# PRBonn/RAP

Hardware: AMD Instinct MI355X
Metric: registered points/sec @20 flow steps, 2-view N=4096 (higher is better)
Workload: dtype f32; 1 GPU; configs[1]: batch=32 samples/GPU x 2 views x 4096 pts, 20 Euler flow steps, rap_12 (d=512, H=8), fp32 (exact-fp32 MFMA), rigidity_forcing=on, final per-view SE(3) fit; preset=1, pairs_per_gpu=32, views=2, points_per_view=4096, flow_steps=20, num_layers=12, rigidity_forcing=True

## Files before the change

rap_amd/csrc/api.hip:

```cpp
#include "../../include/rapflow.h"
#include "half.h"
#include "kernels.h"

#include <mutex>
#include <new>
#include <vector>

static thread_local int g_last_hip_error = 0;
void rap_set_last_hip_error(int e) { g_last_hip_error = e; }

#define RAP_PROF_CLASSES 8
struct ProfRec { hipEvent_t a, b; int cls; };
static std::atomic<bool> g_prof_on{false};
static std::mutex g_prof_mu;
static std::vector<ProfRec> g_prof_recs;
static std::vector<hipEvent_t> g_prof_pool;
static size_t g_prof_pool_used = 0;
static const size_t RAP_PROF_MAX_EVENTS = 1u << 19;

static hipEvent_t prof_event() {
  if (g_prof_pool_used < g_prof_pool.size()) return g_prof_pool[g_prof_pool_used++];
  if (g_prof_pool.size() >= RAP_PROF_MAX_EVENTS) return nullptr;
  hipEvent_t e = nullptr;
  if (hipEventCreate(&e) != hipSuccess) return nullptr;
  g_prof_pool.push_back(e);
  g_prof_pool_used++;
  return e;
}
struct ProfScope {
  hipStream_t s; hipEvent_t a = nullptr, b = nullptr; int cls;
  ProfScope(hipStream_t s_, int cls_) : s(s_), cls(cls_) {
    if (!g_prof_on.load(std::memory_order_relaxed)) return;
    std::lock_guard<std::mutex> lock(g_prof_mu);
    a = prof_event(); b = prof_event();
    if (a && b) (void)hipEventRecord(a, s); else a = b = nullptr;
  }
  ~ProfScope() {
    if (a && b) {
      std::lock_guard<std::mutex> lock(g_prof_mu);
      (void)hipEventRecord(b, s); g_prof_recs.push_back({a, b, cls});
    }
  }
};
extern "C" int rap_profile_enable(int on) { g_prof_on.store(on != 0); return RAP_OK; }
extern "C" int rap_profile_reset(void) { std::lock_guard<std::mutex> lock(g_prof_mu); g_prof_recs.clear(); g_prof_pool_used = 0; return RAP_OK; }
extern "C" int rap_profile_collect_ex(float* h_ms_out, int64_t* h_count_out, int32_t n_classes) {
  if (!h_ms_out || !h_count_out || n_classes <= 0) return RAP_ERR_INVALID;
  std::lock_guard<std::mutex> lock(g_prof_mu);
  for (int c = 0; c < n_classes; ++c) { h_ms_out[c] = 0.f; h_count_out[c] = 0; }
  for (const ProfRec& r : g_prof_recs) {
    if (r.cls >= n_classes) continue;
    if (hipEventSynchronize(r.b) != hipSuccess) return RAP_ERR_HIP;
    float ms = 0.f;
    if (hipEventElapsedTime(&ms, r.a, r.b) != hipSuccess) return RAP_ERR_HIP;
    h_ms_out[r.cls] += ms; h_count_out[r.cls] += 1;
  }
  return RAP_OK;
}
extern "C" int rap_profile_collect(float* h_ms_out, int64_t* h_count_out) { return rap_profile_collect_ex(h_ms_out, h_count_out, 3); }

struct LayerW {
  const float* Wqkv[2];
  const float* Wout[2];
  const float* bout[2];
  const float* gq[2];
  const float* gk[2];
  const float* ffn_g;
  const float* ffn_b;
  const float* Wff1p;
  const float* bff1p;
  const float* Wff2;
  const float* bff2;
};

struct LayerWH {
  const u16* Wqkv[2];
  const u16* Wout[2];
  const u16* Wff1p;
  const u16* Wff2;
  float s_qkv[2] = {1.f, 1.f}, s_out[2] = {1.f, 1.f}, s_ff1 = 1.f, s_ff2 = 1.f;
  float g_v[2] = {1.f, 1.f}, g_ff1 = 1.f;
};
struct HalfWeights {
  u16* blob = nullptr;
  std::vector<LayerWH> layers;
};
#define RAP_MAX_LOGIT_BOUND 40.0f

struct rap_model {
  rap_model_desc desc;
  int d, L, H, F, E;
  int Din = 0;
  int Ks = 128;
  int dtype = RAP_DT_F32;
  bool qk_norm = true;
  int resid_dtype = RAP_DT_F32;
  HalfWeights half[4];
  float* logit_bound = nullptr;
  std::vector<uint8_t> bounded;
  int n_bounded = 0;
  float* raw = nullptr;
  float* derived = nullptr;
  const float* anchor_emb;
  const float* emb_bias;
  const float* Wstatic;
  const float* Wx;
  const float *adaW1, *adab1, *adaW2, *adab2, *adaW3, *adab3;
  std::vector<LayerW> layers;
  const float *hW0, *hb0, *hW2, *hb2, *hW4;
  mutable std::mutex cfg_mu;
};

static bool desc_ok(const rap_model_desc* d) {
  if (!d) return false;
  if (d->embed_dim <= 0 || d->embed_dim % 256 != 0 || d->embed_dim > 1024) return false;
  if (d->num_heads * 64 != d->embed_dim) return false;
  if (d->num_layers <= 0 || d->num_layers > 64) return false;
  if (d->local_feat_dim < 0 || d->local_feat_dim % 4 != 0 || d->local_feat_dim > 40) return false;
  return true;
}

extern rap_tuning_t g_rap_gemm_variant;
extern rap_tuning_t g_rap_gemm_stagger;
extern rap_tuning_t g_rap_gemm_splitk;
extern rap_tuning_t g_rap_geglu_fast;
extern rap_tuning_t g_rap_attn_split;
extern rap_tuning_t g_rap_gemm_h16_variant;
extern rap_tuning_t g_rap_attn_h16_variant;
extern rap_tuning_t g_rap_gemm_h16_persistent;
extern rap_tuning_t g_rap_attn_h16_dma;
extern rap_tuning_t g_rap_gemm_f32_persistent;
extern rap_tuning_t g_rap_attn_x2_wpe;
extern rap_tuning_t g_rap_attn_h16_small;
rap_tuning_t g_rap_attn_lpt = 1;
rap_tuning_t g_rap_x2_min_rows = 1024;
rap_tuning_t g_rap_small_fused = 1;
extern rap_tuning_t g_rap_ring_blocks;
rap_tuning_t g_rap_fuse_qknorm = 1;
extern "C" int rap_set_tuning(int32_t key, int32_t value) {
#ifdef RAP_ABLATION_BUILD
  if (key == 0 && (value == 16 || value == 32 || value == 48)) { g_rap_gemm_variant = value; return RAP_OK; }
  if (key == 2 && (value == 0 || value == 1 || value == 14)) { g_rap_gemm_h16_variant = value; return RAP_OK; }
  if (key == 3 && (value == 0 || value == 5)) { g_rap_attn_h16_variant = value; return RAP_OK; }
  if (key == 4 && value >= 0 && value <= 2) { g_rap_gemm_stagger = value; return RAP_OK; }
#endif
  if (key == 5 && (value == 0 || value == 1)) { g_rap_attn_split = value; return RAP_OK; }
  if (key == 6 && (value == 0 || value == 1)) { g_rap_gemm_splitk = value; return RAP_OK; }
  if (key == 7 && (value == 0 || value == 1)) { g_rap_fuse_qknorm = value; return RAP_OK; }
  if (key == 9 && (value == 0 || value == 1)) { g_rap_geglu_fast = value; return RAP_OK; }
  if (key == 11 && (value == 0 || value == 1)) { g_rap_gemm_h16_persistent = value; return RAP_OK; }
  if (key == 12 && (value == 0 || value == 1)) { g_rap_gemm_f32_persistent = value; return RAP_OK; }
  if (key == 13 && (value == 0 || value == 1)) { g_rap_attn_h16_dma = value; return RAP_OK; }
  if (key == 15 && (value == 0 || value == 1)) { g_rap_attn_lpt = value; return RAP_OK; }
  if (key == 17 && value >= 0) { g_rap_x2_min_rows = value; return RAP_OK; }
  if (key == 18 && value >= 0) { g_rap_ring_blocks = value; return RAP_OK; }
  if (key == 19 && (value == 0 || value == 1)) { g_rap_small_fused = value; return RAP_OK; }
  if (key == 20 && (value == 0 || value == 1 || value == 2 || value == 64 || value == 128 || value == 66 || value == 130)) { g_rap_attn_h16_small = value; return RAP_OK; }
  if (key == 16 && (value == 2 || value == 4)) { g_rap_attn_x2_wpe = value; return RAP_OK; }
  return RAP_ERR_INVALID;
}

extern "C" int rap_version(void) { return RAPFLOW_ABI_VERSION; }
extern "C" int rap_last_hip_error(void) { return g_last_hip_error; }

static bool in_dim_ok(int32_t in_dim) { return in_dim >= 0 && in_dim <= 512 && in_dim % 4 == 0; }
extern "C" int64_t rap_weight_count(const rap_model_desc* desc) { return rap_weight_count_latent(desc, 0); }
extern "C" int64_t rap_weight_count_latent(const rap_model_desc* desc, int32_t in_dim) {
  if (!desc_ok(desc) || !in_dim_ok(in_dim)) return -1;
  const int64_t d = desc->embed_dim, L = desc->num_layers, H = desc->num_heads, E = 147 + desc->local_feat_dim + in_dim;
  int64_t n = 2 * d + d * E + d;
  const int64_t attn = (d * 256 + d) + (d * d + d) + (2 * d * d + 2 * d) + 3 * d * d + (d * d + d) + 2 * H * 64;
  const int64_t layer = 2 * attn + 2 * d + (8 * d * d + 8 * d) + (4 * d * d + d);
  n += L * layer;
  n += (d * d + d) + (d / 2 * d + d / 2) + 3 * (d / 2);
  return n;
}

static int ensure_logit_bounds(rap_model* m, hipStream_t stream);

extern "C" int rap_model_create(const rap_model_desc* desc, const float* d_weights, int64_t n_floats, void* stream_,
                                rap_model** out) {
  return rap_model_create_latent(desc, 0, d_weights, n_floats, stream_, out);
}
extern "C" int rap_model_create_latent(const rap_model_desc* desc, int32_t in_dim, const float* d_weights, int64_t n_floats, void* stream_,
                                       rap_model** out) {
  if (!out) return RAP_ERR_INVALID;
  *out = nullptr;
  if (!desc_ok(desc) || !in_dim_ok(in_dim) || !d_weights) return RAP_ERR_INVALID;
  if (n_floats != rap_weight_count_latent(desc, in_dim)) return RAP_ERR_INVALID;
  hipStream_t stream = (hipStream_t)stream_;
  rap_model* m = new (std::nothrow) rap_model();
  if (!m) return RAP_ERR_ALLOC;
  m->desc = *desc;
  const int d = m->d = desc->embed_dim, L = m->L = desc->num_layers, H = m->H = desc->num_heads;
  m->F = desc->local_feat_dim;
  m->Din = in_dim;
  const int Ks = m->Ks = 128 + (in_dim + 31) / 32 * 32;
  const int E = m->E = 147 + m->F + m->Din;
  if (hipMalloc((void**)&m->raw, (size_t)n_floats * sizeof(float)) != hipSuccess) { delete m; return RAP_ERR_ALLOC; }
  const size_t n_ada = (size_t)2 * L * ((size_t)d * 256 + d + (size_t)d * d + d + (size_t)2 * d * d + 2 * d);
  const size_t n_ff1 = (size_t)L * ((size_t)8 * d * d + 8 * d);
  const size_t n_derived = (size_t)d * Ks + (size_t)d * 64 + n_ada + n_ff1;
  if (hipMalloc((void**)&m->derived, n_derived * sizeof(float)) != hipSuccess) {
    (void)hipFree(m->raw); delete m; return RAP_ERR_ALLOC;
  }
  int rc = RAP_OK;
  auto fail = [&](int code) { rap_model_destroy(m); return code; };
  if (hipMemcpyAsync(m->raw, d_weights, (size_t)n_floats * sizeof(float), hipMemcpyDeviceToDevice, stream) != hipSuccess)
    return fail(RAP_ERR_HIP);

  const float* p = m->raw;
  auto take = [&](size_t n) { const float* r = p; p += n; return r; };
  m->anchor_emb = take((size_t)2 * d);
  const float* embW = take((size_t)d * E);
  m->emb_bias = take(d);

  float* q = m->derived;
  auto carve = [&](size_t n) { float* r = q; q += n; return r; };
  float* Wstatic = carve((size_t)d * Ks);
  float* Wx = carve((size_t)d * 64);
  float* aW1 = carve((size_t)2 * L * d * 256); float* ab1 = carve((size_t)2 * L * d);
  float* aW2 = carve((size_t)2 * L * d * d);   float* ab2 = carve((size_t)2 * L * d);
  float* aW3 = carve((size_t)2 * L * 2 * d * d); float* ab3 = carve((size_t)2 * L * 2 * d);
  m->Wstatic = Wstatic; m->Wx = Wx;
  m->adaW1 = aW1; m->adab1 = ab1; m->adaW2 = aW2; m->adab2 = ab2; m->adaW3 = aW3; m->adab3 = ab3;

  if ((rc = launch_fill_zero(stream, Wstatic, (size_t)d * Ks))) return fail(rc);
  if ((rc = launch_fill_zero(stream, Wx, (size_t)d * 64))) return fail(rc);
  if ((rc = launch_copy_cols(stream, embW, E, 0, Wstatic, Ks, 0, d, 63))) return fail(rc);
  if ((rc = launch_copy_cols(stream, embW, E, 126, Wstatic, Ks, 63, d, 21))) return fail(rc);
  if ((rc = launch_copy_cols(stream, embW, E, 147, Wstatic, Ks, 84, d, m->F))) return fail(rc);
  if ((rc = launch_copy_cols(stream, embW, E, 147 + m->F, Wstatic, Ks, 128, d, m->Din))) return fail(rc);
  if ((rc = launch_copy_cols(stream, embW, E, 63, Wx, 64, 0, d, 63))) return fail(rc);

  m->layers.resize(L);
  for (int i = 0; i < L; ++i) {
    LayerW& lw = m->layers[i];
    for (int a = 0; a < 2; ++a) {
      const int j = 2 * i + a;
      const float* W1 = take((size_t)d * 256); const float* b1 = take(d);
      const float* W2 = take((size_t)d * d);   const float* b2 = take(d);
      const float* W3 = take((size_t)2 * d * d); const float* b3 = take((size_t)2 * d);
      if ((rc = launch_copy_cols(stream, W1, 256, 0, aW1 + (size_t)j * d * 256, 256, 0, d, 256))) return fail(rc);
      if ((rc = launch_copy_cols(stream, b1, d, 0, ab1 + (size_t)j * d, d, 0, 1, d))) return fail(rc);
      if ((rc = launch_copy_cols(stream, W2, d, 0, aW2 + (size_t)j * d * d, d, 0, d, d))) return fail(rc);
      if ((rc = launch_copy_cols(stream, b2, d, 0, ab2 + (size_t)j * d, d, 0, 1, d))) return fail(rc);
      if ((rc = launch_copy_cols(stream, W3, d, 0, aW3 + (size_t)j * 2 * d * d, d, 0, 2 * d, d))) return fail(rc);
      if ((rc = launch_copy_cols(stream, b3, 2 * d, 0, ab3 + (size_t)j * 2 * d, 2 * d, 0, 1, 2 * d))) return fail(rc);
      lw.Wqkv[a] = take((size_t)3 * d * d);
      lw.Wout[a] = take((size_t)d * d);
      lw.bout[a] = take(d);
      lw.gq[a] = take((size_t)H * 64);
      lw.gk[a] = take((size_t)H * 64);
    }
    lw.ffn_g = take(d);
    lw.ffn_b = take(d);
    const float* Wff1 = take((size_t)8 * d * d);
    const float* bff1 = take((size_t)8 * d);
    float* Wp = carve((size_t)8 * d * d);
    float* bp = carve((size_t)8 * d);
    if ((rc = launch_geglu_interleave(stream, Wff1, bff1, Wp, bp, 4 * d, d))) return fail(rc);
    lw.Wff1p = Wp; lw.bff1p = bp;
    lw.Wff2 = take((size_t)d * 4 * d);
    lw.bff2 = take(d);
  }
  m->hW0 = take((size_t)d * d); m->hb0 = take(d);
  m->hW2 = take((size_t)(d / 2) * d); m->hb2 = take(d / 2);
  m->hW4 = take((size_t)3 * (d / 2));
  if ((int64_t)(p - m->raw) != n_floats || (size_t)(q - m->derived) != n_derived) return fail(RAP_ERR_INVALID);
  if ((rc = ensure_logit_bounds(m, stream))) return fail(rc);
  *out = m;
  return RAP_OK;
}

extern "C" void rap_model_destroy(rap_model* m) {
  if (!m) return;
  if (m->raw) (void)hipFree(m->raw);
  if (m->derived) (void)hipFree(m->derived);
  for (int i = 0; i < 4; ++i)
    if (m->half[i].blob) (void)hipFree(m->half[i].blob);
  if (m->logit_bound) (void)hipFree(m->logit_bound);
  delete m;
}

static int ensure_logit_bounds(rap_model* m, hipStream_t stream) {
  if (m->logit_bound) return RAP_OK;
  const int n = m->L * 2 * m->H;
  if (hipMalloc((void**)&m->logit_bound, (size_t)n * sizeof(float)) != hipSuccess) { m->logit_bound = nullptr; return RAP_ERR_ALLOC; }
  for (int i = 0; i < m->L; ++i)
    for (int a = 0; a < 2; ++a) {
      const int rc = launch_qk_logit_bound(stream, m->layers[i].gq[a], m->layers[i].gk[a], m->H, m->logit_bound + (size_t)(2 * i + a) * m->H);
      if (rc) return rc;
    }
  std::vector<float> hb(n);
  RAP_HIP_CHECK(hipMemcpyAsync(hb.data(), m->logit_bound, (size_t)n * sizeof(float), hipMemcpyDeviceToHost, stream));
  RAP_HIP_CHECK(hipStreamSynchronize(stream));
  m->bounded.assign((size_t)2 * m->L, 1);
  for (int j = 0; j < 2 * m->L; ++j)
    for (int h = 0; h < m->H; ++h)
      if (!(hb[(size_t)j * m->H + h] <= RAP_MAX_LOGIT_BOUND)) m->bounded[j] = 0;
  m->n_bounded = 0;
  for (uint8_t b : m->bounded) m->n_bounded += b;
  return RAP_OK;
}

static int build_x2_weights(rap_model* m, hipStream_t stream) {
  HalfWeights& hw = m->half[RAP_DT_F32X2];
  const size_t d = m->d, L = m->L;
  const size_t per_layer = 2 * (2 * (3 * d * d + d * d) + 8 * d * d + 4 * d * d);
  const int nt = (int)(6 * L);
// ... 1242 lines not shown
```

rap_amd/csrc/attn_f32.hip:

```cpp
#include "kernels.h"

#define AQ_WAVE 64
#define AKV 64
#define KLD 68
#define VLD 64
#define ATTN_FENCE __builtin_amdgcn_sched_barrier(0x406);

__device__ __forceinline__ float xhalf_max(float v) {
  const auto r = __builtin_amdgcn_permlane32_swap(__float_as_uint(v), __float_as_uint(v), false, false);
  return fmaxf(__uint_as_float(r[0]), __uint_as_float(r[1]));
}
__device__ __forceinline__ float xhalf_sum(float v) {
  const auto r = __builtin_amdgcn_permlane32_swap(__float_as_uint(v), __float_as_uint(v), false, false);
  return __uint_as_float(r[0]) + __uint_as_float(r[1]);
}

#define ATTN_DEFER_THR 11.5f
__device__ __forceinline__ float amax3(float a, float b, float c) {
  float r;
  asm("v_max3_f32 %0, %1, %2, %3" : "=v"(r) : "v"(a), "v"(b), "v"(c));
  return r;
}

template <int NW, bool BOUNDED, bool SPLIT = false>
__global__ __launch_bounds__(64 * NW, 2) void attention_f32_kernel(const float* __restrict__ qkv, float* __restrict__ out,
                                                                  int TP, int heads, const AttnWorkItem* __restrict__ items,
                                                                  const float* __restrict__ bound, float* __restrict__ part_o,
                                                                  float* __restrict__ part_l) {
  __shared__ __attribute__((aligned(16))) float smem[2 * AKV * KLD + 2 * AKV * VLD];
  float* Ks = smem;
  float* Vs = smem + 2 * AKV * KLD;

  const int head = blockIdx.x % heads;
  const AttnWorkItem it = items[blockIdx.x / heads];
  const int len = it.seg_len;
  if (len <= 0) return;
  const int tid = threadIdx.x;
  const int lane = tid & 63, wave = tid >> 6;
  const int hi = lane >> 5, l31 = lane & 31;

  const size_t plane = (size_t)heads * TP * 64;
  const float* Qg = qkv + ((size_t)head * TP + it.seg_start) * 64;
  const float* Kg = Qg + plane;
  const float* Vg = Qg + 2 * plane;

  const int qw0 = it.q0 + wave * AQ_WAVE;
  const bool wave_active = qw0 < len;
  if (NW == 8) {
    if (__builtin_amdgcn_readfirstlane(threadIdx.x) >= 256) __builtin_amdgcn_s_setprio(1);
  }

  const float qscale = 0.125f * 1.44269504088896340736f;
  float qf[2][32];
#pragma unroll
  for (int qt = 0; qt < 2; ++qt) {
    int q = qw0 + qt * 32 + l31;
    q = q < len ? q : len - 1;
    const float* qp = Qg + (size_t)q * 64 + 4 * hi;
#pragma unroll
    for (int g = 0; g < 8; ++g) {
      const float4 v = *reinterpret_cast<const float4*>(qp + 8 * g);
      qf[qt][g * 4 + 0] = v.x * qscale;
      qf[qt][g * 4 + 1] = v.y * qscale;
      qf[qt][g * 4 + 2] = v.z * qscale;
      qf[qt][g * 4 + 3] = v.w * qscale;
    }
  }

  f32x16 o[2][2];
#pragma unroll
  for (int a = 0; a < 2; ++a)
#pragma unroll
    for (int b = 0; b < 2; ++b)
#pragma unroll
      for (int r = 0; r < 16; ++r) o[a][b][r] = 0.f;
  const bool bound_ok = BOUNDED ? (bound[head] <= 40.0f) : true;
  float mrun[2] = {-1e30f, -1e30f};
  float lsum[2] = {0.f, 0.f};

  constexpr int RS = 4 * NW;
  const int srow = tid >> 4;
  const int sc4 = (tid & 15) * 4;
  float4 rk0, rk1, rk2, rk3, rv0, rv1, rv2, rv3;
  const int nkv = (len + AKV - 1) / AKV;
  int t_begin = 0, t_end = nkv;
  if (SPLIT) {
    t_begin = (int)((long)nkv * blockIdx.y / gridDim.y);
    t_end = (int)((long)nkv * (blockIdx.y + 1) / gridDim.y);
  }
  const int koff = srow * KLD + sc4;
  const int voff = srow * VLD + sc4;

#define ATTN_LOAD_ONE(T, I, RK, RV)                                          \
  {                                                                          \
    int key_ = (T) * AKV + srow + RS * (I);                                  \
    key_ = key_ < len ? key_ : len - 1;                                      \
    RK = *reinterpret_cast<const float4*>(Kg + (size_t)key_ * 64 + sc4);     \
    RV = *reinterpret_cast<const float4*>(Vg + (size_t)key_ * 64 + sc4);     \
  }
#define ATTN_LOAD_TILE(T)          \
  ATTN_LOAD_ONE(T, 0, rk0, rv0)    \
  ATTN_LOAD_ONE(T, 1, rk1, rv1)    \
  if constexpr (NW == 4) {         \
    ATTN_LOAD_ONE(T, 2, rk2, rv2)  \
    ATTN_LOAD_ONE(T, 3, rk3, rv3)  \
  }
#define ATTN_STORE_ONE(BUF, I, RK, RV)                                                            \
  *reinterpret_cast<float4*>(&Ks[(BUF) * (AKV * KLD) + koff + RS * (I) * KLD]) = RK;              \
  *reinterpret_cast<float4*>(&Vs[(BUF) * (AKV * VLD) + voff + RS * (I) * VLD]) = RV;
#define ATTN_STORE_TILE(BUF)           \
  ATTN_STORE_ONE(BUF, 0, rk0, rv0)     \
  ATTN_STORE_ONE(BUF, 1, rk1, rv1)     \
  if constexpr (NW == 4) {             \
    ATTN_STORE_ONE(BUF, 2, rk2, rv2)   \
    ATTN_STORE_ONE(BUF, 3, rk3, rv3)   \
  }

  ATTN_LOAD_TILE(t_begin)
  ATTN_STORE_TILE(0)
  __syncthreads();

  for (int t = t_begin; t < t_end; ++t) {
    const int cur = (t - t_begin) & 1;
    const bool more = (t + 1) < t_end;
    if (more) { ATTN_LOAD_TILE(t + 1) }

    if (wave_active) {
      const float* Kc = Ks + cur * (AKV * KLD);
      const float* Vc = Vs + cur * (AKV * VLD);
#pragma unroll
      for (int kt = 0; kt < 2; ++kt) {
        const int kbase = t * AKV + kt * 32;
        if (kbase >= len) break;
        f32x16 st[2];
#pragma unroll
        for (int r = 0; r < 16; ++r) { st[0][r] = 0.f; st[1][r] = 0.f; }
        const float* kp = Kc + (kt * 32 + l31) * KLD + 4 * hi;
        const float* vp = Vc + (kt * 32 + 4 * hi) * VLD + 2 * l31;
        float4 kf = *reinterpret_cast<const float4*>(kp);
        float2 vfa, vfb;
#pragma unroll
        for (int g = 0; g < 8; ++g) {
          float4 kn = kf;
          if (g < 7) kn = *reinterpret_cast<const float4*>(kp + 8 * (g + 1));
          else { vfa = *reinterpret_cast<const float2*>(vp); vfb = *reinterpret_cast<const float2*>(vp + VLD); }
          ATTN_FENCE
          st[0] = __builtin_amdgcn_mfma_f32_32x32x2f32(kf.x, qf[0][g * 4 + 0], st[0], 0, 0, 0);
          st[1] = __builtin_amdgcn_mfma_f32_32x32x2f32(kf.x, qf[1][g * 4 + 0], st[1], 0, 0, 0);
          st[0] = __builtin_amdgcn_mfma_f32_32x32x2f32(kf.y, qf[0][g * 4 + 1], st[0], 0, 0, 0);
          st[1] = __builtin_amdgcn_mfma_f32_32x32x2f32(kf.y, qf[1][g * 4 + 1], st[1], 0, 0, 0);
          st[0] = __builtin_amdgcn_mfma_f32_32x32x2f32(kf.z, qf[0][g * 4 + 2], st[0], 0, 0, 0);
          st[1] = __builtin_amdgcn_mfma_f32_32x32x2f32(kf.z, qf[1][g * 4 + 2], st[1], 0, 0, 0);
          st[0] = __builtin_amdgcn_mfma_f32_32x32x2f32(kf.w, qf[0][g * 4 + 3], st[0], 0, 0, 0);
          st[1] = __builtin_amdgcn_mfma_f32_32x32x2f32(kf.w, qf[1][g * 4 + 3], st[1], 0, 0, 0);
          ATTN_FENCE
          kf = kn;
        }
        if (kbase + 32 > len) {
#pragma unroll
          for (int r = 0; r < 16; ++r) {
            const bool valid = (kbase + mfma32_crow(r, hi)) < len;
            st[0][r] = valid ? st[0][r] : -1e30f;
            st[1][r] = valid ? st[1][r] : -1e30f;
          }
        }
        if (BOUNDED) {
#pragma unroll
          for (int qt = 0; qt < 2; ++qt) {
            float pa = 0.f, pb2 = 0.f;
#pragma unroll
            for (int r = 0; r < 16; r += 2) {
              const float e0 = __builtin_amdgcn_exp2f(st[qt][r]);
              const float e1 = __builtin_amdgcn_exp2f(st[qt][r + 1]);
              st[qt][r] = e0; st[qt][r + 1] = e1;
              pa += e0; pb2 += e1;
            }
            lsum[qt] += pa + pb2;
          }
        } else {
#pragma unroll
        for (int qt = 0; qt < 2; ++qt) {
          float mx = amax3(st[qt][0], st[qt][1], st[qt][2]);
#pragma unroll
          for (int r = 3; r < 15; r += 2) mx = amax3(mx, st[qt][r], st[qt][r + 1]);
          mx = xhalf_max(fmaxf(mx, st[qt][15]));
          if (__builtin_amdgcn_ballot_w64(mx > mrun[qt] + ATTN_DEFER_THR) != 0) {
            const float mnew = fmaxf(mrun[qt], mx);
            const float alpha = __builtin_amdgcn_exp2f(mrun[qt] - mnew);
            mrun[qt] = mnew;
            lsum[qt] *= alpha;
#pragma unroll
            for (int r = 0; r < 16; ++r) {
              o[qt][0][r] *= alpha;
              o[qt][1][r] *= alpha;
            }
          }
          float pa = 0.f, pb2 = 0.f;
#pragma unroll
          for (int r = 0; r < 16; r += 2) {
            const float e0 = __builtin_amdgcn_exp2f(st[qt][r] - mrun[qt]);
            const float e1 = __builtin_amdgcn_exp2f(st[qt][r + 1] - mrun[qt]);
            st[qt][r] = e0; st[qt][r + 1] = e1;
            pa += e0; pb2 += e1;
          }
          lsum[qt] += pa + pb2;
        }
        }
#pragma unroll
        for (int r = 0; r < 16; r += 2) {
          float2 vna = vfa, vnb = vfb;
          if (r + 2 < 16) {
            const int k0 = ((r + 2) & 3) + 8 * ((r + 2) >> 2);
            const int k1 = ((r + 3) & 3) + 8 * ((r + 3) >> 2);
            vna = *reinterpret_cast<const float2*>(vp + k0 * VLD);
            vnb = *reinterpret_cast<const float2*>(vp + k1 * VLD);
          }
          ATTN_FENCE
          o[0][0] = __builtin_amdgcn_mfma_f32_32x32x2f32(vfa.x, st[0][r], o[0][0], 0, 0, 0);
          o[0][1] = __builtin_amdgcn_mfma_f32_32x32x2f32(vfa.y, st[0][r], o[0][1], 0, 0, 0);
          o[1][0] = __builtin_amdgcn_mfma_f32_32x32x2f32(vfa.x, st[1][r], o[1][0], 0, 0, 0);
          o[1][1] = __builtin_amdgcn_mfma_f32_32x32x2f32(vfa.y, st[1][r], o[1][1], 0, 0, 0);
          o[0][0] = __builtin_amdgcn_mfma_f32_32x32x2f32(vfb.x, st[0][r + 1], o[0][0], 0, 0, 0);
          o[0][1] = __builtin_amdgcn_mfma_f32_32x32x2f32(vfb.y, st[0][r + 1], o[0][1], 0, 0, 0);
          o[1][0] = __builtin_amdgcn_mfma_f32_32x32x2f32(vfb.x, st[1][r + 1], o[1][0], 0, 0, 0);
          o[1][1] = __builtin_amdgcn_mfma_f32_32x32x2f32(vfb.y, st[1][r + 1], o[1][1], 0, 0, 0);
          ATTN_FENCE
          vfa = vna; vfb = vnb;
        }
      }
    }

    if (more) { ATTN_STORE_TILE(cur ^ 1) }
    __syncthreads();
  }

  if (!wave_active) return;
  const int dmodel = heads * 64;
#pragma unroll
  for (int qt = 0; qt < 2; ++qt) {
    const int q = qw0 + qt * 32 + l31;
    const float ltot = xhalf_sum(lsum[qt]);
    const float inv = SPLIT ? 1.0f : (bound_ok ? 1.0f / ltot : __builtin_nanf(""));
    if (q < len) {
      float* op = (SPLIT ? part_o + (size_t)blockIdx.y * TP * dmodel : out) + (size_t)(it.seg_start + q) * dmodel + head * 64;
      if (SPLIT && hi == 0)
        part_l[((size_t)blockIdx.y * TP + it.seg_start + q) * heads + head] = bound_ok ? ltot : __builtin_nanf("");
#pragma unroll
      for (int rg = 0; rg < 4; ++rg) {
        const int d0 = 2 * (8 * rg + 4 * hi);
        float4 w0, w1;
        w0.x = o[qt][0][4 * rg + 0] * inv; w0.y = o[qt][1][4 * rg + 0] * inv;
        w0.z = o[qt][0][4 * rg + 1] * inv; w0.w = o[qt][1][4 * rg + 1] * inv;
        w1.x = o[qt][0][4 * rg + 2] * inv; w1.y = o[qt][1][4 * rg + 2] * inv;
        w1.z = o[qt][0][4 * rg + 3] * inv; w1.w = o[qt][1][4 * rg + 3] * inv;
        *reinterpret_cast<float4*>(op + d0) = w0;
        *reinterpret_cast<float4*>(op + d0 + 4) = w1;
      }
    }
  }
}

#define WL_THREADS 1024
#define WL_TILE 4096
#define WL_SORT_MAX 8192
__device__ __forceinline__ int wl_len(const int32_t* __restrict__ cu, int s) { const int l = cu[s + 1] - cu[s]; return l > 0 ? l : 0; }
__global__ __launch_bounds__(WL_THREADS) void build_attn_worklist_kernel(const int32_t* __restrict__ cu, int nseg, AttnWorkItem* __restrict__ items,
                                                                          int max_items, int bq, int32_t* __restrict__ sort_ws) {
  if (blockIdx.x != 0) return;
  const int tid = threadIdx.x;
  const AttnWorkItem none = {0, 0, 0, 0};
  if (!sort_ws) {
    if (tid != 0) return;
    int n = 0;
    for (int s = 0; s < nseg; ++s) {
      const int a = cu[s], len = wl_len(cu, s);
      for (int q0 = 0; q0 < len && n < max_items; q0 += bq) { const AttnWorkItem w = {a, len, q0, 0}; items[n++] = w; }
    }
    for (; n < max_items; ++n) items[n] = none;
    return;
  }
  __shared__ int lens[WL_TILE];
  __shared__ int partial[WL_THREADS];
  __shared__ int total_items;
  int32_t* order = sort_ws;
  if (nseg > WL_SORT_MAX) {
    for (int s = tid; s < nseg; s += WL_THREADS) order[s] = s;
  } else
  for (int s0 = 0; s0 < nseg; s0 += WL_THREADS) {
    const int s = s0 + tid;
    const int my = s < nseg ? wl_len(cu, s) : -1;
    int rank = 0;
    for (int j0 = 0; j0 < nseg; j0 += WL_TILE) {
      __syncthreads();
      for (int j = tid; j < WL_TILE && j0 + j < nseg; j += WL_THREADS) lens[j] = wl_len(cu, j0 + j);
      __syncthreads();
      const int nj = nseg - j0 < WL_TILE ? nseg - j0 : WL_TILE;
      if (s < nseg)
        for (int j = 0; j < nj; ++j) rank += (lens[j] > my || (lens[j] == my && j0 + j < s)) ? 1 : 0;
    }
    if (s < nseg) order[rank] = s;
  }
  __threadfence_block();
  __syncthreads();
  const int per = (nseg + WL_THREADS - 1) / WL_THREADS;
  const int r0 = tid * per, r1 = (r0 + per) < nseg ? (r0 + per) : nseg;
  int sum = 0;
  for (int r = r0; r < r1; ++r) { const int sg = order[r]; sum += (wl_len(cu, sg) + bq - 1) / bq; }
  partial[tid] = sum;
  __syncthreads();
  if (tid == 0) {
    int acc = 0;
    for (int t = 0; t < WL_THREADS; ++t) { const int v = partial[t]; partial[t] = acc; acc += v; }
    total_items = acc;
  }
  __syncthreads();
  int n = partial[tid];
  for (int r = r0; r < r1; ++r) {
    const int sg = order[r];
    const int a = cu[sg], len = wl_len(cu, sg);
    for (int q0 = 0; q0 < len; q0 += bq, ++n)
      if (n < max_items) { const AttnWorkItem w = {a, len, q0, 0}; items[n] = w; }
  }
  __syncthreads();
  const int total = total_items < 0 ? 0 : total_items < max_items ? total_items : max_items;
  for (int i = total + tid; i < max_items; i += WL_THREADS) items[i] = none;
}

rap_tuning_t g_rap_attn_variant = 1;
rap_tuning_t g_rap_attn_split = 1;
static int attn_block_queries() { return RAP_ATTN_BQ; }

int launch_build_attn_worklist(hipStream_t stream, const int32_t* cu_seqlens, int nseg, AttnWorkItem* items,
                               int max_items, int block_queries, int32_t* sort_ws) {
  if (max_items <= 0) return RAP_OK;
  hipLaunchKernelGGL(build_attn_worklist_kernel, dim3(1), dim3(WL_THREADS), 0, stream, cu_seqlens, nseg, items, max_items,
                     block_queries > 0 ? block_queries : attn_block_queries(), sort_ws);
  RAP_LAUNCH_CHECK();
  return RAP_OK;
}

__global__ __launch_bounds__(256) void attention_combine_kernel(const float* __restrict__ part_o, const float* __restrict__ part_l,
                                                                float* __restrict__ out, int TP, int heads, int splits,
                                                                const int32_t* __restrict__ cover_cu, int cover_nseg) {
  const int dmodel = heads * 64;
  const long i = (long)blockIdx.x * 256 + threadIdx.x;
  if (i >= (long)TP * dmodel / 4) return;
  const long t = i / (dmodel / 4);
  const int c = (int)(i % (dmodel / 4)) * 4;
  if (cover_cu && (t < cover_cu[0] || t >= cover_cu[cover_nseg])) {
    *reinterpret_cast<float4*>(out + t * dmodel + c) = float4{0.f, 0.f, 0.f, 0.f};
    return;
  }
  float4 acc = {0.f, 0.f, 0.f, 0.f};
  float l = 0.f;
  for (int s = 0; s < splits; ++s) {
    const float4 v = *reinterpret_cast<const float4*>(part_o + ((size_t)s * TP + t) * dmodel + c);
    acc.x += v.x; acc.y += v.y; acc.z += v.z; acc.w += v.w;
    l += part_l[((size_t)s * TP + t) * heads + (c >> 6)];
  }
  const float inv = l > 0.f ? 1.0f / l : 0.f;
  acc.x *= inv; acc.y *= inv; acc.z *= inv; acc.w *= inv;
  *reinterpret_cast<float4*>(out + t * dmodel + c) = acc;
}

int attention_f32_splits(int max_items, int heads, bool bounded) {
  if (!bounded || g_rap_attn_split == 0) return 1;
  const long blocks = (long)max_items * heads;
  return blocks <= 160 ? 4 : blocks <= 320 ? 2 : 1;
}

int launch_attention_f32(hipStream_t stream, const float* qkv, float* out, int TP, int heads, const AttnWorkItem* items,
                         int max_items, const float* bound, float* part_o, float* part_l, int splits, const int32_t* cover_cu,
                         int cover_nseg) {
  if (max_items <= 0 || TP <= 0) return RAP_OK;
  if (heads <= 0) return RAP_ERR_INVALID;
  if (splits > 1) {
    if (!bound || !part_o || !part_l) return RAP_ERR_INVALID;
    unsigned dyn = 0;
    if ((long)max_items * heads * splits <= 384) {
      dyn = 16384;
      if (hipFuncSetAttribute(reinterpret_cast<const void*>(attention_f32_kernel<4, true, true>), hipFuncAttributeMaxDynamicSharedMemorySize, dyn) != hipSuccess) {
        rap_set_last_hip_error((int)hipGetLastError());
        return RAP_ERR_HIP;
      }
    }
    hipLaunchKernelGGL((attention_f32_kernel<4, true, true>), dim3(max_items * heads, splits), dim3(256), dyn, stream, qkv, out, TP,
                       heads, items, bound, part_o, part_l);
    RAP_LAUNCH_CHECK();
    const long n4 = (long)TP * heads * 16;
    hipLaunchKernelGGL(attention_combine_kernel, dim3((unsigned)((n4 + 255) / 256)), dim3(256), 0, stream, part_o, part_l, out, TP,
                       heads, splits, cover_cu, cover_nseg);
    RAP_LAUNCH_CHECK();
    return RAP_OK;
  }
  float* const no = nullptr;
  if (bound) hipLaunchKernelGGL((attention_f32_kernel<4, true>), dim3(max_items * heads), dim3(256), 0, stream, qkv, out, TP, heads, items, bound, no, no);
  else hipLaunchKernelGGL((attention_f32_kernel<4, false>), dim3(max_items * heads), dim3(256), 0, stream, qkv, out, TP, heads, items, bound, no, no);
  RAP_LAUNCH_CHECK();
  return RAP_OK;
}
```

Before: 16370 points/s.

## Use direct global-to-LDS DMA with swizzled K tiles and optional software-pipelined attention

Replaces the register-staged K/V tile loads and LDS stores in the fp32 attention kernel with global_load_lds_dwordx4 DMA. K rows use an XOR swizzle instead of padding (KLD 68→64), and the split-kernel dynamic LDS size is adjusted. It also adds an optional PIPE variant that interleaves the softmax of one 32-key subtile with the QK and PV MFMAs of the neighbour using sched_group_barrier. The PIPE path is off by default, but the DMA and swizzle path runs by default and removes register staging and VGPR pressure. The risk is extra m0 manipulation and vmcnt waits before each barrier.

```diff
diff --git a/rap_amd/csrc/api.hip b/rap_amd/csrc/api.hip
--- a/rap_amd/csrc/api.hip
+++ b/rap_amd/csrc/api.hip
@@ -125,6 +125,7 @@
 extern rap_tuning_t g_rap_gemm_splitk;
 extern rap_tuning_t g_rap_geglu_fast;
 extern rap_tuning_t g_rap_attn_split;
+extern rap_tuning_t g_rap_attn_f32_pipe;
 extern rap_tuning_t g_rap_gemm_h16_variant;
 extern rap_tuning_t g_rap_attn_h16_variant;
 extern rap_tuning_t g_rap_gemm_h16_persistent;
@@ -156,6 +157,7 @@
   if (key == 18 && value >= 0) { g_rap_ring_blocks = value; return RAP_OK; }
   if (key == 19 && (value == 0 || value == 1)) { g_rap_small_fused = value; return RAP_OK; }
   if (key == 20 && (value == 0 || value == 1 || value == 2 || value == 64 || value == 128 || value == 66 || value == 130)) { g_rap_attn_h16_small = value; return RAP_OK; }
+  if (key == 22 && (value == 0 || value == 1)) { g_rap_attn_f32_pipe = value; return RAP_OK; }
   if (key == 16 && (value == 2 || value == 4)) { g_rap_attn_x2_wpe = value; return RAP_OK; }
   return RAP_ERR_INVALID;
 }
diff --git a/rap_amd/csrc/attn_f32.hip b/rap_amd/csrc/attn_f32.hip
--- a/rap_amd/csrc/attn_f32.hip
+++ b/rap_amd/csrc/attn_f32.hip
@@ -2,9 +2,11 @@
 
 #define AQ_WAVE 64
 #define AKV 64
-#define KLD 68
+#define KLD 64
 #define VLD 64
 #define ATTN_FENCE __builtin_amdgcn_sched_barrier(0x406);
+#define ATTN_PHASE __builtin_amdgcn_sched_barrier(0);
+#define ATTN_SGB(MASK, N) __builtin_amdgcn_sched_group_barrier((MASK), (N), 0);
 
 __device__ __forceinline__ float xhalf_max(float v) {
   const auto r = __builtin_amdgcn_permlane32_swap(__float_as_uint(v), __float_as_uint(v), false, false);
@@ -13,6 +15,11 @@
 __device__ __forceinline__ float xhalf_sum(float v) {
   const auto r = __builtin_amdgcn_permlane32_swap(__float_as_uint(v), __float_as_uint(v), false, false);
   return __uint_as_float(r[0]) + __uint_as_float(r[1]);
+}
+__device__ __forceinline__ float sadd(float a, float b) {
+  float r = a + b;
+  asm("" : "+v"(r));
+  return r;
 }
 
 #define ATTN_DEFER_THR 11.5f
@@ -22,7 +29,7 @@
   return r;
 }
 
-template <int NW, bool BOUNDED, bool SPLIT = false>
+template <int NW, bool BOUNDED, bool SPLIT = false, bool PIPE = false>
 __global__ __launch_bounds__(64 * NW, 2) void attention_f32_kernel(const float* __restrict__ qkv, float* __restrict__ out,
                                                                   int TP, int heads, const AttnWorkItem* __restrict__ items,
                                                                   const float* __restrict__ bound, float* __restrict__ part_o,
@@ -79,159 +86,196 @@
   float lsum[2] = {0.f, 0.f};
 
   constexpr int RS = 4 * NW;
+  constexpr int NP = 16 / NW;
   const int srow = tid >> 4;
-  const int sc4 = (tid & 15) * 4;
-  float4 rk0, rk1, rk2, rk3, rv0, rv1, rv2, rv3;
+  const int kls = ((tid & 15) ^ (srow & 15)) * 4;
+  const int vls = (tid & 15) * 4;
   const int nkv = (len + AKV - 1) / AKV;
   int t_begin = 0, t_end = nkv;
   if (SPLIT) {
     t_begin = (int)((long)nkv * blockIdx.y / gridDim.y);
     t_end = (int)((long)nkv * (blockIdx.y + 1) / gridDim.y);
   }
-  const int koff = srow * KLD + sc4;
-  const int voff = srow * VLD + sc4;
-
-#define ATTN_LOAD_ONE(T, I, RK, RV)                                          \
-  {                                                                          \
-    int key_ = (T) * AKV + srow + RS * (I);                                  \
-    key_ = key_ < len ? key_ : len - 1;                                      \
-    RK = *reinterpret_cast<const float4*>(Kg + (size_t)key_ * 64 + sc4);     \
-    RV = *reinterpret_cast<const float4*>(Vg + (size_t)key_ * 64 + sc4);     \
-  }
-#define ATTN_LOAD_TILE(T)          \
-  ATTN_LOAD_ONE(T, 0, rk0, rv0)    \
-  ATTN_LOAD_ONE(T, 1, rk1, rv1)    \
-  if constexpr (NW == 4) {         \
-    ATTN_LOAD_ONE(T, 2, rk2, rv2)  \
-    ATTN_LOAD_ONE(T, 3, rk3, rv3)  \
-  }
-#define ATTN_STORE_ONE(BUF, I, RK, RV)                                                            \
-  *reinterpret_cast<float4*>(&Ks[(BUF) * (AKV * KLD) + koff + RS * (I) * KLD]) = RK;              \
-  *reinterpret_cast<float4*>(&Vs[(BUF) * (AKV * VLD) + voff + RS * (I) * VLD]) = RV;
-#define ATTN_STORE_TILE(BUF)           \
-  ATTN_STORE_ONE(BUF, 0, rk0, rv0)     \
-  ATTN_STORE_ONE(BUF, 1, rk1, rv1)     \
-  if constexpr (NW == 4) {             \
-    ATTN_STORE_ONE(BUF, 2, rk2, rv2)   \
-    ATTN_STORE_ONE(BUF, 3, rk3, rv3)   \
-  }
-
-  ATTN_LOAD_TILE(t_begin)
-  ATTN_STORE_TILE(0)
-  __syncthreads();
+  const unsigned lds_k = __builtin_amdgcn_readfirstlane((unsigned)(size_t)(__attribute__((address_space(3))) float*)Ks + (unsigned)wave * 1024u);
+  const unsigned lds_v = __builtin_amdgcn_readfirstlane((unsigned)(size_t)(__attribute__((address_space(3))) float*)Vs + (unsigned)wave * 1024u);
+
+#define ATTN_DMA1(GSRC, LDSB)                                                                                 \
+  {                                                                                                           \
+    unsigned keep_;                                                                                           \
+    asm volatile("s_mov_b32 %0, m0\n\ts_mov_b32 m0, %2\n\ts_nop 0\n\tglobal_load_lds_dwordx4 %1, off\n\ts_mov_b32 m0, %0" \
+                 : "=&s"(keep_) : "v"(GSRC), "s"(LDSB) : "memory");                                           \
+  }
+#define ATTN_DMA_TILE(T, BUF)                                                                                 \
+  _Pragma("unroll") for (int i_ = 0; i_ < NP; ++i_) {                                                         \
+    int key_ = (T) * AKV + srow + RS * i_;                                                                    \
+    key_ = key_ < len ? key_ : len - 1;                                                                       \
+    ATTN_DMA1(Kg + (size_t)key_ * 64 + kls, lds_k + (unsigned)((BUF) * (AKV * KLD) + i_ * (NW * 64 * 4)) * 4u) \
+    ATTN_DMA1(Vg + (size_t)key_ * 64 + vls, lds_v + (unsigned)((BUF) * (AKV * VLD) + i_ * (NW * 64 * 4)) * 4u) \
+  }
+#define ATTN_SYNC asm volatile("s_waitcnt vmcnt(0)" ::: "memory"); __syncthreads();
+
+  const int swz = l31 & 15;
+  auto s_phase = [&](const float* Kc, const float* Vc, int kt, f32x16 (&st)[2], float2& vfa, float2& vfb, auto fill) {
+#pragma unroll
+    for (int r = 0; r < 16; ++r) { st[0][r] = 0.f; st[1][r] = 0.f; }
+    const float* kp = Kc + (kt * 32 + l31) * KLD;
+    const float* vp = Vc + (kt * 32 + 4 * hi) * VLD + 2 * l31;
+    float4 kf = *reinterpret_cast<const float4*>(kp + ((0 + hi) ^ swz) * 4);
+#pragma unroll
+    for (int g = 0; g < 8; ++g) {
+      float4 kn = kf;
+      if (g < 7) kn = *reinterpret_cast<const float4*>(kp + ((2 * (g + 1) + hi) ^ swz) * 4);
+      else { vfa = *reinterpret_cast<const float2*>(vp); vfb = *reinterpret_cast<const float2*>(vp + VLD); }
+      ATTN_FENCE
+      st[0] = __builtin_amdgcn_mfma_f32_32x32x2f32(kf.x, qf[0][g * 4 + 0], st[0], 0, 0, 0);
+      st[1] = __builtin_amdgcn_mfma_f32_32x32x2f32(kf.x, qf[1][g * 4 + 0], st[1], 0, 0, 0);
+      st[0] = __builtin_amdgcn_mfma_f32_32x32x2f32(kf.y, qf[0][g * 4 + 1], st[0], 0, 0, 0);
+      st[1] = __builtin_amdgcn_mfma_f32_32x32x2f32(kf.y, qf[1][g * 4 + 1], st[1], 0, 0, 0);
+      st[0] = __builtin_amdgcn_mfma_f32_32x32x2f32(kf.z, qf[0][g * 4 + 2], st[0], 0, 0, 0);
+      st[1] = __builtin_amdgcn_mfma_f32_32x32x2f32(kf.z, qf[1][g * 4 + 2], st[1], 0, 0, 0);
+      st[0] = __builtin_amdgcn_mfma_f32_32x32x2f32(kf.w, qf[0][g * 4 + 3], st[0], 0, 0, 0);
+      st[1] = __builtin_amdgcn_mfma_f32_32x32x2f32(kf.w, qf[1][g * 4 + 3], st[1], 0, 0, 0);
+      fill();
+      ATTN_FENCE
+      kf = kn;
+    }
+  };
+  auto pv_phase = [&](const float* Vc, int kt, f32x16 (&st)[2], float2 vfa, float2 vfb, auto fill) {
+    const float* vp = Vc + (kt * 32 + 4 * hi) * VLD + 2 * l31;
+#pragma unroll
+    for (int r = 0; r < 16; r += 2) {
+      float2 vna = vfa, vnb = vfb;
+      if (r + 2 < 16) {
+        const int k0 = ((r + 2) & 3) + 8 * ((r + 2) >> 2);
+        const int k1 = ((r + 3) & 3) + 8 * ((r + 3) >> 2);
+        vna = *reinterpret_cast<const float2*>(vp + k0 * VLD);
+        vnb = *reinterpret_cast<const float2*>(vp + k1 * VLD);
+      }
+      ATTN_FENCE
+      o[0][0] = __builtin_amdgcn_mfma_f32_32x32x2f32(vfa.x, st[0][r], o[0][0], 0, 0, 0);
+      o[0][1] = __builtin_amdgcn_mfma_f32_32x32x2f32(vfa.y, st[0][r], o[0][1], 0, 0, 0);
+      o[1][0] = __builtin_amdgcn_mfma_f32_32x32x2f32(vfa.x, st[1][r], o[1][0], 0, 0, 0);
+      o[1][1] = __builtin_amdgcn_mfma_f32_32x32x2f32(vfa.y, st[1][r], o[1][1], 0, 0, 0);
+      o[0][0] = __builtin_amdgcn_mfma_f32_32x32x2f32(vfb.x, st[0][r + 1], o[0][0], 0, 0, 0);
+      o[0][1] = __builtin_amdgcn_mfma_f32_32x32x2f32(vfb.y, st[0][r + 1], o[0][1], 0, 0, 0);
+      o[1][0] = __builtin_amdgcn_mfma_f32_32x32x2f32(vfb.x, st[1][r + 1], o[1][0], 0, 0, 0);
+      o[1][1] = __builtin_amdgcn_mfma_f32_32x32x2f32(vfb.y, st[1][r + 1], o[1][1], 0, 0, 0);
+      fill();
+      ATTN_FENCE
+      vfa = vna; vfb = vnb;
+    }
+  };
+  auto no_fill = [] {};
+  auto fill = [] {
+#pragma unroll
+    for (int j = 0; j < 4; ++j) {
+      if constexpr (BOUNDED) { ATTN_SGB(0x008, 1) ATTN_SGB(0x400, 1) ATTN_SGB(0x008, 1) ATTN_SGB(0x002, 1) }
+      else { ATTN_SGB(0x008, 1) ATTN_SGB(0x400, 1) ATTN_SGB(0x002, 1) ATTN_SGB(0x008, 1) ATTN_SGB(0x002, 2) }
+    }
+  };
+  auto mask = [&](int kbase, f32x16 (&st)[2]) {
+    if (kbase + 32 > len) {
+#pragma unroll
+      for (int r = 0; r < 16; ++r) {
+        const bool valid = (kbase + mfma32_crow(r, hi)) < len;
+        st[0][r] = valid ? st[0][r] : -1e30f;
+        st[1][r] = valid ? st[1][r] : -1e30f;
+      }
+    }
+  };
+  auto softmax = [&](f32x16 (&st)[2], float (&psum)[2], bool (&grow)[2], float (&mold)[2]) {
+#pragma unroll
+    for (int qt = 0; qt < 2; ++qt) {
+      float m = 0.f;
+      if (!BOUNDED) {
+        float mx = amax3(st[qt][0], st[qt][1], st[qt][2]);
+#pragma unroll
+        for (int r = 3; r < 15; r += 2) mx = amax3(mx, st[qt][r], st[qt][r + 1]);
+        mx = xhalf_max(fmaxf(mx, st[qt][15]));
+        grow[qt] = __builtin_amdgcn_ballot_w64(mx > mrun[qt] + ATTN_DEFER_THR) != 0;
+        mold[qt] = mrun[qt];
+        mrun[qt] = grow[qt] ? fmaxf(mrun[qt], mx) : mrun[qt];
+        m = mrun[qt];
+      }
+      float pa = 0.f, pb2 = 0.f;
+#pragma unroll
+      for (int r = 0; r < 16; r += 2) {
+        const float e0 = __builtin_amdgcn_exp2f(BOUNDED ? st[qt][r] : st[qt][r] - m);
+        const float e1 = __builtin_amdgcn_exp2f(BOUNDED ? st[qt][r + 1] : st[qt][r + 1] - m);
+        st[qt][r] = e0; st[qt][r + 1] = e1;
+        pa = sadd(pa, e0); pb2 = sadd(pb2, e1);
+      }
+      psum[qt] = pa + pb2;
+    }
+  };
+  auto rescale = [&](const float (&psum)[2], const bool (&grow)[2], const float (&mold)[2]) {
+#pragma unroll
+    for (int qt = 0; qt < 2; ++qt) {
+      if (!BOUNDED && grow[qt]) {
+        const float alpha = __builtin_amdgcn_exp2f(mold[qt] - mrun[qt]);
+        lsum[qt] *= alpha;
+#pragma unroll
+        for (int r = 0; r < 16; ++r) {
+          o[qt][0][r] *= alpha;
+          o[qt][1][r] *= alpha;
+        }
+      }
+      lsum[qt] += psum[qt];
+    }
+  };
+
+  ATTN_DMA_TILE(t_begin, 0)
+  ATTN_SYNC
 
   for (int t = t_begin; t < t_end; ++t) {
     const int cur = (t - t_begin) & 1;
-    const bool more = (t + 1) < t_end;
-    if (more) { ATTN_LOAD_TILE(t + 1) }
+    if ((t + 1) < t_end) { ATTN_DMA_TILE(t + 1, cur ^ 1) }
 
     if (wave_active) {
       const float* Kc = Ks + cur * (AKV * KLD);
       const float* Vc = Vs + cur * (AKV * VLD);
-#pragma unroll
-      for (int kt = 0; kt < 2; ++kt) {
-        const int kbase = t * AKV + kt * 32;
-        if (kbase >= len) break;
-        f32x16 st[2];
-#pragma unroll
-        for (int r = 0; r < 16; ++r) { st[0][r] = 0.f; st[1][r] = 0.f; }
-        const float* kp = Kc + (kt * 32 + l31) * KLD + 4 * hi;
-        const float* vp = Vc + (kt * 32 + 4 * hi) * VLD + 2 * l31;
-        float4 kf = *reinterpret_cast<const float4*>(kp);
-        float2 vfa, vfb;
-#pragma unroll
-        for (int g = 0; g < 8; ++g) {
-          float4 kn = kf;
-          if (g < 7) kn = *reinterpret_cast<const float4*>(kp + 8 * (g + 1));
-          else { vfa = *reinterpret_cast<const float2*>(vp); vfb = *reinterpret_cast<const float2*>(vp + VLD); }
-          ATTN_FENCE
-          st[0] = __builtin_amdgcn_mfma_f32_32x32x2f32(kf.x, qf[0][g * 4 + 0], st[0], 0, 0, 0);
-          st[1] = __builtin_amdgcn_mfma_f32_32x32x2f32(kf.x, qf[1][g * 4 + 0], st[1], 0, 0, 0);
-          st[0] = __builtin_amdgcn_mfma_f32_32x32x2f32(kf.y, qf[0][g * 4 + 1], st[0], 0, 0, 0);
-          st[1] = __builtin_amdgcn_mfma_f32_32x32x2f32(kf.y, qf[1][g * 4 + 1], st[1], 0, 0, 0);
-          st[0] = __builtin_amdgcn_mfma_f32_32x32x2f32(kf.z, qf[0][g * 4 + 2], st[0], 0, 0, 0);
-          st[1] = __builtin_amdgcn_mfma_f32_32x32x2f32(kf.z, qf[1][g * 4 + 2], st[1], 0, 0, 0);
-          st[0] = __builtin_amdgcn_mfma_f32_32x32x2f32(kf.w, qf[0][g * 4 + 3], st[0], 0, 0, 0);
-          st[1] = __builtin_amdgcn_mfma_f32_32x32x2f32(kf.w, qf[1][g * 4 + 3], st[1], 0, 0, 0);
-          ATTN_FENCE
-          kf = kn;
+      const int kbase = t * AKV;
+      if (PIPE) {
+        f32x16 s0[2], s1[2];
+        float2 va0, vb0, va1, vb1;
+        float ps0[2], ps1[2], al0[2], al1[2];
+        bool gr0[2], gr1[2];
+        ATTN_PHASE
+        s_phase(Kc, Vc, 0, s0, va0, vb0, no_fill);
+        ATTN_PHASE
+        mask(kbase, s0);
+        ATTN_PHASE
+        softmax(s0, ps0, gr0, al0);
+        s_phase(Kc, Vc, 1, s1, va1, vb1, fill);
+        ATTN_PHASE
+        rescale(ps0, gr0, al0);
+        mask(kbase + 32, s1);
+        ATTN_PHASE
+        softmax(s1, ps1, gr1, al1);
+        pv_phase(Vc, 0, s0, va0, vb0, fill);
+        ATTN_PHASE
+        rescale(ps1, gr1, al1);
+        ATTN_PHASE
+        pv_phase(Vc, 1, s1, va1, vb1, no_fill);
+        ATTN_PHASE
+      } else {
+#pragma unroll
+        for (int kt = 0; kt < 2; ++kt) {
+          if (kbase + kt * 32 >= len) break;
+          f32x16 st[2];
+          float2 vfa, vfb;
+          float ps[2], al[2];
+          bool gr[2];
+          s_phase(Kc, Vc, kt, st, vfa, vfb, no_fill);
+          mask(kbase + kt * 32, st);
+          softmax(st, ps, gr, al);
+          rescale(ps, gr, al);
+          pv_phase(Vc, kt, st, vfa, vfb, no_fill);
         }
-        if (kbase + 32 > len) {
-#pragma unroll
-          for (int r = 0; r < 16; ++r) {
-            const bool valid = (kbase + mfma32_crow(r, hi)) < len;
-            st[0][r] = valid ? st[0][r] : -1e30f;
-            st[1][r] = valid ? st[1][r] : -1e30f;
-          }
-        }
-        if (BOUNDED) {
-#pragma unroll
-          for (int qt = 0; qt < 2; ++qt) {
-            float pa = 0.f, pb2 = 0.f;
-#pragma unroll
-            for (int r = 0; r < 16; r += 2) {
-              const float e0 = __builtin_amdgcn_exp2f(st[qt][r]);
-              const float e1 = __builtin_amdgcn_exp2f(st[qt][r + 1]);
-              st[qt][r] = e0; st[qt][r + 1] = e1;
-              pa += e0; pb2 += e1;
-            }
-            lsum[qt] += pa + pb2;
-          }
-        } else {
-#pragma unroll
-        for (int qt = 0; qt < 2; ++qt) {
-          float mx = amax3(st[qt][0], st[qt][1], st[qt][2]);
-#pragma unroll
-          for (int r = 3; r < 15; r += 2) mx = amax3(mx, st[qt][r], st[qt][r + 1]);
-          mx = xhalf_max(fmaxf(mx, st[qt][15]));
-          if (__builtin_amdgcn_ballot_w64(mx > mrun[qt] + ATTN_DEFER_THR) != 0) {
-            const float mnew = fmaxf(mrun[qt], mx);
-            const float alpha = __builtin_amdgcn_exp2f(mrun[qt] - mnew);
-            mrun[qt] = mnew;
-            lsum[qt] *= alpha;
-#pragma unroll
-            for (int r = 0; r < 16; ++r) {
-              o[qt][0][r] *= alpha;
-              o[qt][1][r] *= alpha;
-            }
-          }
-          float pa = 0.f, pb2 = 0.f;
-#pragma unroll
-          for (int r = 0; r < 16; r += 2) {
-            const float e0 = __builtin_amdgcn_exp2f(st[qt][r] - mrun[qt]);
-            const float e1 = __builtin_amdgcn_exp2f(st[qt][r + 1] - mrun[qt]);
-            st[qt][r] = e0; st[qt][r + 1] = e1;
-            pa += e0; pb2 += e1;
-          }
-          lsum[qt] += pa + pb2;
-        }
-        }
-#pragma unroll
-        for (int r = 0; r < 16; r += 2) {
-          float2 vna = vfa, vnb = vfb;
-          if (r + 2 < 16) {
-            const int k0 = ((r + 2) & 3) + 8 * ((r + 2) >> 2);
-            const int k1 = ((r + 3) & 3) + 8 * ((r + 3) >> 2);
-            vna = *reinterpret_cast<const float2*>(vp + k0 * VLD);
-            vnb = *reinterpret_cast<const float2*>(vp + k1 * VLD);
-          }
-          ATTN_FENCE
-          o[0][0] = __builtin_amdgcn_mfma_f32_32x32x2f32(vfa.x, st[0][r], o[0][0], 0, 0, 0);
-          o[0][1] = __builtin_amdgcn_mfma_f32_32x32x2f32(vfa.y, st[0][r], o[0][1], 0, 0, 0);
-          o[1][0] = __builtin_amdgcn_mfma_f32_32x32x2f32(vfa.x, st[1][r], o[1][0], 0, 0, 0);
-          o[1][1] = __builtin_amdgcn_mfma_f32_32x32x2f32(vfa.y, st[1][r], o[1][1], 0, 0, 0);
-          o[0][0] = __builtin_amdgcn_mfma_f32_32x32x2f32(vfb.x, st[0][r + 1], o[0][0], 0, 0, 0);
-          o[0][1] = __builtin_amdgcn_mfma_f32_32x32x2f32(vfb.y, st[0][r + 1], o[0][1], 0, 0, 0);
-          o[1][0] = __builtin_amdgcn_mfma_f32_32x32x2f32(vfb.x, st[1][r + 1], o[1][0], 0, 0, 0);
-          o[1][1] = __builtin_amdgcn_mfma_f32_32x32x2f32(vfb.y, st[1][r + 1], o[1][1], 0, 0, 0);
-          ATTN_FENCE
-          vfa = vna; vfb = vnb;
-        }
-      }
-    }
-
-    if (more) { ATTN_STORE_TILE(cur ^ 1) }
-    __syncthreads();
+      }
+    }
+
+    ATTN_SYNC
   }
 
   if (!wave_active) return;
@@ -328,6 +372,7 @@
 
 rap_tuning_t g_rap_attn_variant = 1;
 rap_tuning_t g_rap_attn_split = 1;
+rap_tuning_t g_rap_attn_f32_pipe = 0;
 static int attn_block_queries() { return RAP_ATTN_BQ; }
 
 int launch_build_attn_worklist(hipStream_t stream, const int32_t* cu_seqlens, int nseg, AttnWorkItem* items,
@@ -374,18 +419,25 @@
                          int cover_nseg) {
   if (max_items <= 0 || TP <= 0) return RAP_OK;
   if (heads <= 0) return RAP_ERR_INVALID;
+  const bool pipe = g_rap_attn_f32_pipe != 0;
   if (splits > 1) {
     if (!bound || !part_o || !part_l) return RAP_ERR_INVALID;
+    const void* fn = pipe ? reinterpret_cast<const void*>(attention_f32_kernel<4, true, true, true>)
+                          : reinterpret_cast<const void*>(attention_f32_kernel<4, true, true, false>);
     unsigned dyn = 0;
     if ((long)max_items * heads * splits <= 384) {
-      dyn = 16384;
-      if (hipFuncSetAttribute(reinterpret_cast<const void*>(attention_f32_kernel<4, true, true>), hipFuncAttributeMaxDynamicSharedMemorySize, dyn) != hipSuccess) {
+      dyn = 18432;
+      if (hipFuncSetAttribute(fn, hipFuncAttributeMaxDynamicSharedMemorySize, dyn) != hipSuccess) {
         rap_set_last_hip_error((int)hipGetLastError());
         return RAP_ERR_HIP;
       }
     }
-    hipLaunchKernelGGL((attention_f32_kernel<4, true, true>), dim3(max_items * heads, splits), dim3(256), dyn, stream, qkv, out, TP,
-                       heads, items, bound, part_o, part_l);
+    if (pipe)
+      hipLaunchKernelGGL((attention_f32_kernel<4, true, true, true>), dim3(max_items * heads, splits), dim3(256), dyn, stream, qkv, out,
+                         TP, heads, items, bound, part_o, part_l);
+    else
+      hipLaunchKernelGGL((attention_f32_kernel<4, true, true, false>), dim3(max_items * heads, splits), dim3(256), dyn, stream, qkv, out,
+                         TP, heads, items, bound, part_o, part_l);
     RAP_LAUNCH_CHECK();
     const long n4 = (long)TP * heads * 16;
     hipLaunchKernelGGL(attention_combine_kernel, dim3((unsigned)((n4 + 255) / 256)), dim3(256), 0, stream, part_o, part_l, out, TP,
@@ -394,8 +446,14 @@
     return RAP_OK;
   }
   float* const no = nullptr;
-  if (bound) hipLaunchKernelGGL((attention_f32_kernel<4, true>), dim3(max_items * heads), dim3(256), 0, stream, qkv, out, TP, heads, items, bound, no, no);
-  else hipLaunchKernelGGL((attention_f32_kernel<4, false>), dim3(max_items * heads), dim3(256), 0, stream, qkv, out, TP, heads, items, bound, no, no);
+  const dim3 grid(max_items * heads), blk(256);
+  if (bound) {
+    if (pipe) hipLaunchKernelGGL((attention_f32_kernel<4, true, false, true>), grid, blk, 0, stream, qkv, out, TP, heads, items, bound, no, no);
+    else hipLaunchKernelGGL((attention_f32_kernel<4, true, false, false>), grid, blk, 0, stream, qkv, out, TP, heads, items, bound, no, no);
+  } else {
+    if (pipe) hipLaunchKernelGGL((attention_f32_kernel<4, false, false, true>), grid, blk, 0, stream, qkv, out, TP, heads, items, bound, no, no);
+    else hipLaunchKernelGGL((attention_f32_kernel<4, false, false, false>), grid, blk, 0, stream, qkv, out, TP, heads, items, bound, no, no);
+  }
   RAP_LAUNCH_CHECK();
   return RAP_OK;
 }
```

Measured after the change: 16320 points/s (median of 2 runs). Within noise of the previous version (-0.3%).
